# ratschlab/secedo

Hardware: AMD Instinct MI355X
Metric: cell-pair x locus updates/sec (similarity matrix) (higher is better)
Workload: dtype int64; 1 GPU; C3: 8000 cells x 100000 loci; entries=24345058, kept_entries=24223307, reads=23997029, block_cells=128, tiles=2016, normalization=ADD_MIN, max_fragment_length=1000, num_threads=8, parallelism=single GPU, backend=none, world_size=1, rccl_world_size=1

## Files before the change

### secedo_amd/csrc/simmat_kernels.hip

```cpp
#include "simmat_kernels.hpp"

#include <hip/hip_runtime.h>

#include <algorithm>
#include <type_traits>

namespace secedo {

uint32_t counts_split(uint32_t n_tiles);

namespace {

constexpr uint32_t META_PREV_OVF = 1u << 19;
constexpr uint32_t META_NEXT_OVF = 1u << 20;
constexpr uint32_t C_CELL = 127u;
constexpr uint32_t C_BASE_SHIFT = 7;
constexpr uint32_t C_TAIL = 1u << 9;
constexpr uint32_t C_MULTI = 1u << 10;
constexpr uint32_t C_WIDE = 1u << 11;
constexpr int LUT_DIM = 129;
constexpr int SLUT_DIM = 10;
constexpr long long NO_PAIR = (long long)0x8000000000000000ull;

__device__ __forceinline__ double log_add(double a, double b) {
    const double hi = fmax(a, b), lo = fmin(a, b);
    return hi + log1p(exp(lo - hi));
}

#ifdef SECEDO_STAMPS
__device__ __forceinline__ unsigned long long stamp() {
    unsigned long long t;
    asm volatile("s_memtime %0\n\ts_waitcnt lgkmcnt(0)" : "=s"(t)::"memory");
    return t;
}
__device__ __forceinline__ unsigned long long stamp_real() {
    unsigned long long t;
    asm volatile("s_memrealtime %0\n\ts_waitcnt lgkmcnt(0)" : "=s"(t)::"memory");
    return t;
}
#define STAMP(var) __builtin_amdgcn_sched_barrier(0); const unsigned long long var = stamp(); __builtin_amdgcn_sched_barrier(0)
#else
#define STAMP(var)
#endif

__device__ __forceinline__ uint32_t wave_inclusive_scan(uint32_t v) {
    v += __builtin_amdgcn_update_dpp(0u, v, 0x111, 0xF, 0xF, true);
    v += __builtin_amdgcn_update_dpp(0u, v, 0x112, 0xF, 0xF, true);
    v += __builtin_amdgcn_update_dpp(0u, v, 0x114, 0xF, 0xF, true);
    v += __builtin_amdgcn_update_dpp(0u, v, 0x118, 0xF, 0xF, true);
    v += __builtin_amdgcn_update_dpp(0u, v, 0x142, 0xA, 0xF, true);
    v += __builtin_amdgcn_update_dpp(0u, v, 0x143, 0xC, 0xF, true);
    return v;
}

constexpr uint32_t REF_TABLE_MAX = 128;
__device__ __noinline__ long long llr_fixed_device(const SlowPathArgs *sp, uint32_t xs, uint32_t xd, uint32_t cell_a,
                                                   uint32_t cell_b) {
    if (sp->beyond_list) {
        const uint32_t k = atomicAdd(sp->beyond_count, 1u);
        if (k < sp->beyond_cap) sp->beyond_list[k] = make_uint4(cell_a, cell_b, xs, xd);
        return 0ll;
    }
    const LlrModelDev m = sp->model;
    const int scale_log2 = sp->scale_log2;
    const double s = xs, d = xd;
    const double diff = log_add(s * m.ln_u1 + d * m.ln_v1, s * m.ln_u2 + d * m.ln_v2);
    const double same = log_add(s * m.ln_w1 + d * m.ln_z1, s * m.ln_w2 + d * m.ln_z2);
    return llrint(ldexp(diff - same, scale_log2));
}

__device__ __noinline__ long long slow_pair(const SlowPathArgs *sp, uint32_t r1, uint32_t r2,
                                            uint32_t locus, uint32_t cell_a, uint32_t cell_b) {
    const SlowPathArgs a = *sp;
    uint32_t i1 = a.read_off[r1], e1 = a.read_off[r1 + 1];
    uint32_t i2 = a.read_off[r2], e2 = a.read_off[r2 + 1];
    uint32_t xs = 0, xd = 0, first = 0xFFFFFFFFu;
    while (i1 < e1 && i2 < e2) {
        const uint32_t l1 = a.read_locus[i1], l2 = a.read_locus[i2];
        if (l1 == l2) {
            if (first == 0xFFFFFFFFu) first = l1;
            if (a.read_base[i1] == a.read_base[i2]) ++xs; else ++xd;
            ++i1; ++i2;
        } else if (l1 < l2) {
            ++i1;
        } else {
            ++i2;
        }
    }
    if (first != locus) return NO_PAIR;
    return xs + xd <= REF_TABLE_MAX ? a.lut[xs * LUT_DIM + xd] : llr_fixed_device(sp, xs, xd, cell_a, cell_b);
}

__device__ __noinline__ long long pair_value_full(const SlowPathArgs *sp, uint32_t g1, uint32_t g2) {
    const uint4 *entry = sp->entry;
    const uint4 A1 = entry[g1], A2 = entry[g2];
    if (A1.y & A2.y & 0xFFFFu) return NO_PAIR;
    const bool same = (((A1.x ^ A2.x) >> 16) & 3u) == 0u;
    if ((A1.x & A2.x & (META_PREV_OVF | META_NEXT_OVF)) == 0u) {
        const uint32_t shared = (A1.y & A2.y) >> 16;
        const uint32_t x = A1.z ^ A2.z;
        const uint32_t diff = ((x & 0xFFFFu) | (x >> 16)) & shared;
        const uint32_t nd = __popc(diff);
        const uint32_t xd = nd + (same ? 0u : 1u);
        const uint32_t xs = __popc(shared) - nd + (same ? 1u : 0u);
        return sp->lut[xs * LUT_DIM + xd];
    }
    const uint32_t *entry_read = sp->entry_read;
    return slow_pair(sp, entry_read[g1], entry_read[g2], A1.w, A1.x & 0xFFFFu, A2.x & 0xFFFFu);
}


struct TileChunk {
    uint32_t t;
    bool diag;
    uint32_t lane;
    const uint32_t *offI, *offJ;
    uint32_t r_begin, r_end;
    uint32_t row_begin, row_end;
};
template <int THREADS>
__device__ __forceinline__ TileChunk tile_chunk(const AccumulateArgs &a) {
    const uint32_t t_local = a.wg_tile[blockIdx.x];
    const uint32_t t = a.tile_ids ? a.tile_ids[t_local] : a.tile_begin + t_local;
    const uint32_t chunk = blockIdx.x - a.tile_wg_begin[t_local];
    const uint32_t n_chunks_t = a.tile_wg_begin[t_local + 1] - a.tile_wg_begin[t_local];
    const uint32_t I = a.tile_row[t], J = a.tile_col[t];
    const bool diag = (I == J);
    const uint32_t tid = threadIdx.x, lane = tid & 63u;
    const uint32_t *offI = a.blk_off + (size_t)I * a.stride;
    const uint32_t *offJ = a.blk_off + (size_t)J * a.stride;
    uint32_t r_begin = 0, r_end = a.num_ranges;
    uint32_t row_begin = 0u, row_end = 0xFFFFFFFFu;
    if (n_chunks_t > 1u) {
        const uint32_t L = a.stride - 1u;
        const uint32_t e0 = offI[0];
        const unsigned long long n_row = offI[L] - e0;
        row_begin = e0 + (uint32_t)(n_row * chunk / n_chunks_t);
        row_end = e0 + (uint32_t)(n_row * (chunk + 1u) / n_chunks_t);
        uint32_t before = 0, upto = 0;
        for (uint32_t base = 0; base < a.num_ranges; base += THREADS) {
            const uint32_t k = base + tid;
            bool ends_before = false, begins_inside = false;
            if (k < a.num_ranges) {
                ends_before = offI[a.range_off[k + 1u]] <= row_begin;
                begins_inside = offI[a.range_off[k]] < row_end;
            }
            before += (uint32_t)__syncthreads_count(ends_before);
            upto += (uint32_t)__syncthreads_count(begins_inside);
        }
        r_begin = __builtin_amdgcn_readfirstlane(before);
        r_end = __builtin_amdgcn_readfirstlane(upto);
        row_begin = __builtin_amdgcn_readfirstlane(row_begin);
        row_end = __builtin_amdgcn_readfirstlane(row_end);
    }
    return TileChunk{t, diag, lane, offI, offJ, r_begin, r_end, row_begin, row_end};
}

struct RangeCursor {
// ... 284 lines not shown
                            const bool ok = (!TAIL || pp[u] < total) && (both & C_TAIL) == 0u
                                    && ((x & cell_test) != 0u || !diag);
                            upd += ok ? 1u : 0u;
                            const uint32_t cell = (rr[u].x >> 16) + (ww[u] & C_CELL);
                            if (MCAP > 0) {
                                const bool joint = ok && (both & C_MULTI) != 0u;
                                const unsigned long long bal = __ballot(joint);
                                if (bal) {
                                    if (joint) {
                                        const uint32_t slot = n_list + __builtin_amdgcn_mbcnt_hi(
                                                (uint32_t)(bal >> 32), __builtin_amdgcn_mbcnt_lo((uint32_t)bal, 0u));
                                        mlist[slot] = make_uint2(ib + cur * 64u + oo[u], jb + rr[u].y + pp[u]);
                                        mcell[slot] = (uint16_t)cell;
                                    }
                                    n_list += (uint32_t)__popcll(bal);
                                }
                            } else {
                                multi_seen |= ok ? both : 0u;
                            }
                            if ((a.debug & 1u) == 0u && ok && (both & C_MULTI) == 0u) {
                                const bool differ = (x & (3u << C_BASE_SHIFT)) != 0u;
                                atomicAdd(&tile64[cell], (unsigned long long)(differ ? d01 : d10));
                            }
                        }
                    };
                    using two = std::integral_constant<int, 2>;
                    using one = std::integral_constant<int, 1>;
                    if (!(a.debug & 2u)) {
                        uint32_t base = 0;
                        for (; base + 128u <= total; base += 128u) trip(base, two{}, std::false_type{});
                        if (base < total) {
                            if (total - base <= 64u) trip(base, one{}, std::true_type{});
                            else trip(base, two{}, std::true_type{});
                        }
                    }
                    STAMP(t3);
#ifdef SECEDO_STAMPS
                    st_trip += t3 - t2;
                    st_t3 = t3;
#endif
                    const bool any_multi = MCAP == 0 && (multi_seen & C_MULTI) != 0u;
                    if (MCAP == 0 && __ballot(any_multi)) {
                        for (uint32_t p = lane; p < total; p += 64u) {
                            const uint32_t o = owner[p];
                            const uint2 ro = wrec[o];
                            const uint32_t jc = ro.y + p;
                            const uint32_t w = sJ[jc];
                            const uint32_t x = ro.x ^ w, both = ro.x & w;
                            const bool ok = (both & C_TAIL) == 0u && ((x & cell_test) != 0u || !diag);
                            if (ok && (both & C_MULTI) != 0u) {
                                const long long v = pair_value_full(a.slow, ib + cur * 64u + o, jb + jc);
                                const uint32_t cell = (ro.x >> 16) + (w & C_CELL);
                                if (v == NO_PAIR) ++skipped;
                                else atomicAdd(&tile64[cell], (unsigned long long)v);
                            }
                        }
                    }
                    __builtin_amdgcn_wave_barrier();
#ifdef SECEDO_STAMPS
                    { STAMP(t4); st_post += t4 - st_t3; }
#endif
                } else {
                    wrec[lane] = make_uint2(rec & 0xFFFFu, j0 - pex);
                    for (uint32_t win = 0; win < total; win += (uint32_t)HCAP) {
                        const uint32_t wlen = min((uint32_t)HCAP, total - win);
                        const uint32_t f0 = max(pex, win), f1 = min(pin, win + (uint32_t)HCAP);
                        for (uint32_t p = f0; p < f1; ++p) owner[p - win] = (unsigned char)lane;
                        __builtin_amdgcn_fence(__ATOMIC_RELEASE, "wavefront");
                        __builtin_amdgcn_wave_barrier();
                        for (uint32_t q = lane; q < wlen; q += 64u) {
                            const uint32_t o = owner[q];
                            const uint2 ro = wrec[o];
                            const uint32_t jc = ro.y + win + q;
                            pair(ro.x, sJ[jc], ib + cur * 64u + o, jb + jc);
                        }
                        __builtin_amdgcn_wave_barrier();
                    }
                }
                cur = nxt;
                rec = rec_n;
            }
        } else {
            pair_range_from_hbm<B, THREADS, false>(a, tc, la, ib, ie, dst, d10, d01, upd, skipped);
        }
#ifdef SECEDO_STAMPS
        { STAMP(te); st_loop += te - tb3; }
#endif
        const uint32_t upd_all = upd + (lane == 0u ? upd_w : 0u);
        n_updates += upd_all;
        n_pairs += (unsigned long long)upd_all - skipped;
    }
    STAMP(t_le);
    if (MCAP > 0 && n_list) flush_list();
    STAMP(t_fl);
    __syncthreads();
    STAMP(t_eb);

    {
        uint4 *out = reinterpret_cast<uint4 *>(reinterpret_cast<unsigned long long *>(a.slab) + (size_t)blockIdx.x * B * B);
        const uint4 *src = reinterpret_cast<const uint4 *>(tile64);
        for (uint32_t i = tid; i < B * B / 2; i += THREADS) out[i] = src[i];
    }

    STAMP(t_sl);
#ifdef SECEDO_STAMPS
    if (threadIdx.x == 0u && blockIdx.x < 2048u) {
        unsigned long long *w = a.counters + 16 + 2048 + (size_t)blockIdx.x * 8;
        w[0] = ((unsigned long long)__builtin_amdgcn_s_getreg((31 << 11) | 20) << 32)
                | (unsigned)__builtin_amdgcn_s_getreg((31 << 11) | 4);
        w[1] = t_le - t_pro;
        w[2] = t_fl - t_le;
        w[3] = t_eb - t_fl;
        w[4] = t_sl - t_eb;
        w[5] = st_real_begin;
        w[6] = stamp_real();
        w[7] = st_loop;
        a.counters[16 + blockIdx.x] = ((t_sl - st_begin) & 0xFFFFFFFFull) | ((unsigned long long)r_begin << 32)
                | ((unsigned long long)r_end << 44);
    }
#endif
    add_work_counters<WAVES>(a.counters, reinterpret_cast<unsigned long long *>(sJ), n_updates, n_pairs - skipped_list);
#ifdef SECEDO_STAMPS
    if (tid == 0u) {
        atomicAdd(&a.counters[2], st_setup);
        atomicAdd(&a.counters[3], st_fill);
        atomicAdd(&a.counters[4], st_trip);
        atomicAdd(&a.counters[5], st_batches);
        atomicAdd(&a.counters[6], st_trips);
        atomicAdd(&a.counters[7], stamp() - st_begin);
        atomicAdd(&a.counters[8], 1ull);
        atomicAdd(&a.counters[9], st_bar1);
        atomicAdd(&a.counters[10], st_stage);
        atomicAdd(&a.counters[11], st_pref);
        atomicAdd(&a.counters[12], st_post);
        atomicAdd(&a.counters[13], st_loop);
        atomicMax(&a.counters[14], stamp() - st_begin);
    }
#endif
}


constexpr int COUNTS_RING = 256;
constexpr uint32_t IT_J_SHIFT = 9, IT_C_SHIFT = 24, IT_J_MASK = 0x3FFFu, IT_WIDE = 32;
constexpr uint32_t IT_REC_MASK = 0x1FFu;

template <int B, int THREADS, int NCNT>
__device__ __forceinline__ void correct_epilogue(const AccumulateArgs &a, unsigned char *lds, uint32_t t_local,
                                                 const uint32_t (&cnt)[NCNT]);
template <bool WORDS>
__device__ __forceinline__ uint32_t counts_off_at(const uint16_t *sOff, uint32_t l) {
    if constexpr (WORDS) return (reinterpret_cast<const uint32_t *>(sOff)[l] >> IT_J_SHIFT) & IT_J_MASK;
    else return sOff[l];
}
template <int B, int THREADS, int CAPJ, int CAPL, int GROUP, bool WORDS>
__global__ __launch_bounds__(THREADS) void accumulate_counts(const AccumulateArgs a) {
    static_assert(CAPJ <= 16384, "14 bits of column index in an item");
    static_assert(GROUP >= 2 && GROUP <= 4, "group size");
    constexpr uint32_t ROW_WORDS = B + 1;
    constexpr size_t TILE_BYTES = ((size_t)B * ROW_WORDS * 4 + 15) / 16 * 16;
    constexpr int WAVES = THREADS / 64;
    constexpr int JPT = (CAPJ + THREADS - 1) / THREADS;
    constexpr int OPT = (CAPL + 1 + THREADS - 1) / THREADS;
    constexpr int RING = COUNTS_RING;

    extern __shared__ __attribute__((aligned(16))) unsigned char lds_raw[];
    uint32_t *tile32 = reinterpret_cast<uint32_t *>(lds_raw);
    uint32_t *sJ = reinterpret_cast<uint32_t *>(lds_raw + TILE_BYTES);
    uint16_t *sOff = reinterpret_cast<uint16_t *>(sJ + CAPJ);
    uint32_t *ring = reinterpret_cast<uint32_t *>(sOff + (CAPL + 2) * (WORDS ? 2 : 1)) + (threadIdx.x >> 6) * RING;

    const uint32_t t_local = a.wg_tile[blockIdx.x];
    const uint32_t t = a.tile_ids ? a.tile_ids[t_local] : a.tile_begin + t_local;
    const uint32_t chunk = blockIdx.x - a.tile_wg_begin[t_local];
    const uint32_t n_chunks_t = a.tile_wg_begin[t_local + 1] - a.tile_wg_begin[t_local];
    const uint32_t I = a.tile_row[t], J = a.tile_col[t];
    const bool diag = (I == J);
    const uint32_t tid = threadIdx.x, lane = tid & 63u;
    const uint32_t *offI = a.blk_off + (size_t)I * a.stride;
    const uint32_t *offJ = a.blk_off + (size_t)J * a.stride;
    uint32_t r_begin = 0, r_end = a.num_ranges;
    uint32_t row_begin = 0u, row_end = 0xFFFFFFFFu;
    if (n_chunks_t > 1u) {
        const uint32_t L = a.stride - 1u;
        const uint32_t e0 = offI[0];
        const unsigned long long n_row = offI[L] - e0;
        row_begin = e0 + (uint32_t)(n_row * chunk / n_chunks_t);
        row_end = e0 + (uint32_t)(n_row * (chunk + 1u) / n_chunks_t);
        uint32_t before = 0, upto = 0;
        for (uint32_t base = 0; base < a.num_ranges; base += THREADS) {
            const uint32_t k = base + tid;
            bool ends_before = false, begins_inside = false;
            if (k < a.num_ranges) {
                ends_before = offI[a.range_off[k + 1u]] <= row_begin;
                begins_inside = offI[a.range_off[k]] < row_end;
            }
            before += (uint32_t)__syncthreads_count(ends_before);
            upto += (uint32_t)__syncthreads_count(begins_inside);
        }
        r_begin = __builtin_amdgcn_readfirstlane(before);
        r_end = __builtin_amdgcn_readfirstlane(upto);
        row_begin = __builtin_amdgcn_readfirstlane(row_begin);
        row_end = __builtin_amdgcn_readfirstlane(row_end);
    }
    const TileChunk tc{t, diag, lane, offI, offJ, r_begin, r_end, row_begin, row_end};
    for (uint32_t i = tid; i < B * ROW_WORDS; i += THREADS) tile32[i] = 0u;

    unsigned long long n_updates = 0;
    uint32_t upd_w = 0;
    uint32_t ring_head = 0, ring_tail = 0;

    uint32_t pJ[JPT], pI[JPT], pO[OPT];
    uint32_t pO1[WORDS ? OPT : 1];
    RangeCursor nx;
    bool n_staged = false;
    auto prefetch = [&](uint32_t r) {
        nx.advance(a, tc, r);
        n_staged = (nx.je - nx.jb) <= (uint32_t)CAPJ && (nx.ie - nx.ib) <= (uint32_t)CAPJ
                && (nx.lb - nx.la) <= (uint32_t)CAPL;
        if (n_staged) {
            const __amdgpu_buffer_rsrc_t rj = __builtin_amdgcn_make_buffer_rsrc(
                    const_cast<uint32_t *>(a.entry32 + nx.jb), 0, (int)((nx.je - nx.jb) * 4u), 0x00020000);
            const __amdgpu_buffer_rsrc_t ro = __builtin_amdgcn_make_buffer_rsrc(
                    const_cast<uint32_t *>(offJ + nx.la), 0, (int)((nx.lb - nx.la + 1u) * 4u), 0x00020000);
#pragma unroll
            for (int k = 0; k < JPT; ++k)
                pJ[k] = (uint32_t)__builtin_amdgcn_raw_buffer_load_b32(rj, (int)(tid * 4u), k * THREADS * 4, 0);
#pragma unroll
            for (int k = 0; k < OPT; ++k)
                pO[k] = (uint32_t)__builtin_amdgcn_raw_buffer_load_b32(ro, (int)(tid * 4u), k * THREADS * 4, 0);
            if (WORDS) {
#pragma unroll
                for (int k = 0; k < OPT; ++k)
                    pO1[k] = (uint32_t)__builtin_amdgcn_raw_buffer_load_b32(ro, (int)(tid * 4u + 4u), k * THREADS * 4, 0);
            }
        }
    };
    auto prefetch_rows = [&]() {
        if (n_staged) {
            const __amdgpu_buffer_rsrc_t ri = __builtin_amdgcn_make_buffer_rsrc(
                    const_cast<uint32_t *>(a.entry32 + nx.ib), 0, (int)((nx.ie - nx.ib) * 4u), 0x00020000);
#pragma unroll
            for (int k = 0; k < JPT; ++k)
                pI[k] = (uint32_t)__builtin_amdgcn_raw_buffer_load_b32(ri, (int)(tid * 4u), k * THREADS * 4, 0);
        }
    };

    if (r_begin < r_end) {
        nx.prime(a, tc);
        prefetch(r_begin);
        prefetch_rows();
    }
#ifdef SECEDO_STAMPS
    unsigned long long st_barA = 0, st_stage = 0, st_items = 0, st_prim = 0, st_drain = 0, st_nprim = 0, st_ndrain = 0;
    const unsigned long long st_begin = stamp();
#endif
    {
        const bool DIAG = diag;
        const uint32_t lds_base = (uint32_t)reinterpret_cast<uintptr_t>(lds_raw);
        auto pair_slot = [&](uint32_t rec9, uint32_t row_byte, uint32_t w, unsigned long long in) {
            if (DIAG) in &= __ballot((w & 0xFFFFu) != ((rec9 & C_CELL) << 2));
            upd_w += (uint32_t)__popcll(in);
            const uint32_t addr = row_byte + (w & 0xFFFFu);
            if (__builtin_amdgcn_inverse_ballot_w64(in))
                atomicAdd(reinterpret_cast<uint32_t *>(lds_raw + addr),
                          (w >> 16) != (rec9 >> C_BASE_SHIFT) ? 0x10000u : 1u);
        };
        auto pair_slot_asm = [&](uint32_t rbase, uint32_t row_addr, uint32_t w, unsigned long long in) {
            upd_w += (uint32_t)__popcll(in);
            uint32_t addr, val;
            unsigned long long saved;
            asm volatile("s_and_saveexec_b64 %[saved], %[in]\n\t"
                         "v_cmp_eq_u32_sdwa vcc, %[w], %[rb] src0_sel:WORD_1 src1_sel:DWORD\n\t"
                         "v_add_u32_sdwa %[addr], %[row], %[w] dst_sel:DWORD dst_unused:UNUSED_PAD src0_sel:DWORD "
                         "src1_sel:WORD_0\n\t"
                         "s_nop 0\n\t"
                         "v_cndmask_b32_e64 %[val], %[k], 1, vcc\n\t"
                         "ds_add_u32 %[addr], %[val]\n\t"
                         "s_mov_b64 exec, %[saved]"
                         : [saved] "=&s"(saved), [addr] "=&v"(addr), [val] "=&v"(val)
                         : [in] "s"(in), [w] "v"(w), [rb] "v"(rbase), [row] "v"(row_addr), [k] "v"(0x10000u)
                         : "vcc", "memory");
        };

        auto group_load = [&](uint32_t item, uint32_t (&w)[GROUP]) {
            const uint32_t *p = sJ + ((item >> IT_J_SHIFT) & IT_J_MASK);
#pragma unroll
            for (int u = 0; u < GROUP; ++u) w[u] = p[u];
        };
        auto group_pair = [&](uint32_t item, const uint32_t (&w)[GROUP]) {
            const uint32_t c = item >> IT_C_SHIFT;
            const uint32_t rec9 = item & IT_REC_MASK;
            const uint32_t row_byte = (item & C_CELL) * (ROW_WORDS * 4u);
            unsigned long long in[GROUP];
#pragma unroll
            for (int u = 0; u < GROUP; ++u) in[u] = __ballot(c > (uint32_t)u);
            const unsigned long long more = __ballot(c > (uint32_t)GROUP);
            if (!DIAG && (GROUP == 4 || GROUP == 2)) {
                const uint32_t rbase = rec9 >> C_BASE_SHIFT, row_addr = lds_base + row_byte;
#pragma unroll
                for (int u = 0; u < GROUP; ++u) upd_w += (uint32_t)__popcll(in[u]);
                uint32_t a0, a1, a2, a3, v0, v1, v2, v3;
                unsigned long long saved, q0, q1, q2, q3;
                if (GROUP == 4) {
                    asm volatile("v_cmp_eq_u32_sdwa %[q0], %[w0], %[rb] src0_sel:WORD_1 src1_sel:DWORD\n\t"
                                 "v_cmp_eq_u32_sdwa %[q1], %[w1], %[rb] src0_sel:WORD_1 src1_sel:DWORD\n\t"
                                 "v_cmp_eq_u32_sdwa %[q2], %[w2], %[rb] src0_sel:WORD_1 src1_sel:DWORD\n\t"
                                 "v_cmp_eq_u32_sdwa %[q3], %[w3], %[rb] src0_sel:WORD_1 src1_sel:DWORD\n\t"
                                 "v_add_u32_sdwa %[a0], %[row], %[w0] dst_sel:DWORD dst_unused:UNUSED_PAD src0_sel:DWORD src1_sel:WORD_0\n\t"
                                 "v_add_u32_sdwa %[a1], %[row], %[w1] dst_sel:DWORD dst_unused:UNUSED_PAD src0_sel:DWORD src1_sel:WORD_0\n\t"
                                 "v_add_u32_sdwa %[a2], %[row], %[w2] dst_sel:DWORD dst_unused:UNUSED_PAD src0_sel:DWORD src1_sel:WORD_0\n\t"
                                 "v_add_u32_sdwa %[a3], %[row], %[w3] dst_sel:DWORD dst_unused:UNUSED_PAD src0_sel:DWORD src1_sel:WORD_0\n\t"
                                 "v_cndmask_b32_e64 %[v0], %[k], 1, %[q0]\n\t"
                                 "v_cndmask_b32_e64 %[v1], %[k], 1, %[q1]\n\t"
                                 "v_cndmask_b32_e64 %[v2], %[k], 1, %[q2]\n\t"
                                 "v_cndmask_b32_e64 %[v3], %[k], 1, %[q3]\n\t"
                                 "s_mov_b64 %[saved], exec\n\t"
                                 "s_mov_b64 exec, %[in0]\n\t"
                                 "ds_add_u32 %[a0], %[v0]\n\t"
                                 "s_mov_b64 exec, %[in1]\n\t"
                                 "ds_add_u32 %[a1], %[v1]\n\t"
                                 "s_mov_b64 exec, %[in2]\n\t"
                                 "ds_add_u32 %[a2], %[v2]\n\t"
                                 "s_mov_b64 exec, %[in3]\n\t"
                                 "ds_add_u32 %[a3], %[v3]\n\t"
                                 "s_mov_b64 exec, %[saved]"
                                 : [a0] "=&v"(a0), [a1] "=&v"(a1), [a2] "=&v"(a2), [a3] "=&v"(a3), [v0] "=&v"(v0), [v1] "=&v"(v1),
                                   [v2] "=&v"(v2), [v3] "=&v"(v3), [saved] "=&s"(saved), [q0] "=&s"(q0), [q1] "=&s"(q1),
                                   [q2] "=&s"(q2), [q3] "=&s"(q3)
                                 : [w0] "v"(w[0]), [w1] "v"(w[1 % GROUP]), [w2] "v"(w[2 % GROUP]), [w3] "v"(w[3 % GROUP]),
                                   [rb] "v"(rbase), [row] "v"(row_addr), [k] "v"(0x10000u), [in0] "s"(in[0]),
                                   [in1] "s"(in[1 % GROUP]), [in2] "s"(in[2 % GROUP]), [in3] "s"(in[3 % GROUP])
                                 : "memory");
                } else {
                    asm volatile("v_cmp_eq_u32_sdwa %[q0], %[w0], %[rb] src0_sel:WORD_1 src1_sel:DWORD\n\t"
                                 "v_cmp_eq_u32_sdwa %[q1], %[w1], %[rb] src0_sel:WORD_1 src1_sel:DWORD\n\t"
                                 "v_add_u32_sdwa %[a0], %[row], %[w0] dst_sel:DWORD dst_unused:UNUSED_PAD src0_sel:DWORD src1_sel:WORD_0\n\t"
                                 "v_add_u32_sdwa %[a1], %[row], %[w1] dst_sel:DWORD dst_unused:UNUSED_PAD src0_sel:DWORD src1_sel:WORD_0\n\t"
                                 "s_mov_b64 %[saved], exec\n\t"
                                 "v_cndmask_b32_e64 %[v0], %[k], 1, %[q0]\n\t"
                                 "v_cndmask_b32_e64 %[v1], %[k], 1, %[q1]\n\t"
                                 "s_mov_b64 exec, %[in0]\n\t"
                                 "ds_add_u32 %[a0], %[v0]\n\t"
                                 "s_mov_b64 exec, %[in1]\n\t"
                                 "ds_add_u32 %[a1], %[v1]\n\t"
                                 "s_mov_b64 exec, %[saved]"
                                 : [a0] "=&v"(a0), [a1] "=&v"(a1), [v0] "=&v"(v0), [v1] "=&v"(v1), [saved] "=&s"(saved),
                                   [q0] "=&s"(q0), [q1] "=&s"(q1)
                                 : [w0] "v"(w[0]), [w1] "v"(w[1 % GROUP]), [rb] "v"(rbase), [row] "v"(row_addr), [k] "v"(0x10000u),
                                   [in0] "s"(in[0]), [in1] "s"(in[1 % GROUP])
                                 : "memory");
                    (void)a2; (void)a3; (void)v2; (void)v3; (void)q2; (void)q3;
                }
            } else if (!DIAG) {
                const uint32_t rbase = rec9 >> C_BASE_SHIFT, row_addr = lds_base + row_byte;
#pragma unroll
                for (int u = 0; u < GROUP; ++u) pair_slot_asm(rbase, row_addr, w[u], in[u]);
            } else {
#pragma unroll
                for (int u = 0; u < GROUP; ++u) pair_slot(rec9, row_byte, w[u], in[u]);
            }
            if (more) {
                if (__builtin_amdgcn_inverse_ballot_w64(more)) {
                    const uint32_t slot = ring_tail + __builtin_amdgcn_mbcnt_hi(
                            (uint32_t)(more >> 32), __builtin_amdgcn_mbcnt_lo((uint32_t)more, 0u));
                    ring[slot & (RING - 1)] = item + ((uint32_t)GROUP << IT_J_SHIFT) - ((uint32_t)GROUP << IT_C_SHIFT);
                }
                ring_tail += (uint32_t)__popcll(more);
            }
        };
        auto group4 = [&](uint32_t item) {
            uint32_t w[GROUP];
            group_load(item, w);
            group_pair(item, w);
        };
        auto drain_one = [&]() {
            __builtin_amdgcn_fence(__ATOMIC_RELEASE, "wavefront");
            __builtin_amdgcn_wave_barrier();
            const uint32_t n = min(64u, ring_tail - ring_head);
            uint32_t it = 0u;
            if (lane < n) it = ring[(ring_head + lane) & (RING - 1)];
            __builtin_amdgcn_wave_barrier();
            ring_head += n;
            group4(it);
        };

        for (uint32_t r = r_begin; r < r_end; ++r) {
            const uint32_t la = nx.la, ib = nx.ib, ie = nx.ie, jb = nx.jb, dsh = nx.dsh;
            const bool staged = n_staged;
            STAMP(s0);
            __syncthreads();
            STAMP(s1);
            if (staged) {
                static_assert(JPT * THREADS <= CAPJ && OPT * THREADS <= CAPL + 2, "unconditional staging stores");
#pragma unroll
                for (int k = 0; k < JPT; ++k)
                    sJ[tid + k * THREADS] = ((pJ[k] & C_CELL) << 2) | ((pJ[k] << (16 - C_BASE_SHIFT)) & 0x30000u);
                if (WORDS) {
#pragma unroll
                    for (int k = 0; k < OPT; ++k)
                        reinterpret_cast<uint32_t *>(sOff)[tid + k * THREADS] = (((pO[k] - jb) & IT_J_MASK) << IT_J_SHIFT)
                                                | (min(pO1[k] - pO[k], 255u) << IT_C_SHIFT);
                } else {
#pragma unroll
                    for (int k = 0; k < OPT; ++k) sOff[tid + k * THREADS] = (uint16_t)(pO[k] - jb);
                }
            }
            __syncthreads();
            STAMP(s2);

            const uint32_t nI = ie - ib;
            upd_w = 0;
            if (staged) {
                uint32_t item[JPT];
                uint32_t any_wide = 0;
                if (WORDS && !DIAG) {
                    uint32_t word[JPT];
#pragma unroll
                    for (int k = 0; k < JPT; ++k) word[k] = reinterpret_cast<const uint32_t *>(sOff)[pI[k] >> 16];
#pragma unroll
                    for (int k = 0; k < JPT; ++k) {
                        item[k] = tid + k * THREADS < nI ? (pI[k] & IT_REC_MASK) | word[k] : 0u;
                        any_wide |= item[k];
                    }
                    any_wide >>= IT_C_SHIFT;
                } else {
#pragma unroll
                    for (int k = 0; k < JPT; ++k) {
                        const uint32_t i = tid + k * THREADS;
                        const uint32_t rec = pI[k];
                        const uint32_t lrel = rec >> 16;
                        uint32_t j0 = counts_off_at<WORDS>(sOff, lrel);
                        const uint32_t j1 = counts_off_at<WORDS>(sOff, lrel + 1);
                        if (DIAG) j0 = i + dsh + 1u;
                        const uint32_t c = (i < nI && j1 > j0) ? j1 - j0 : 0u;
                        any_wide |= c;
                        item[k] = (rec & IT_REC_MASK) | ((j0 & IT_J_MASK) << IT_J_SHIFT) | (c << IT_C_SHIFT);
                    }
                }
                if (__ballot(any_wide >= IT_WIDE)) {
#pragma unroll
                    for (int k = 0; k < JPT; ++k) {
                        const uint32_t i = tid + k * THREADS;
                        const uint32_t rec = pI[k];
                        const uint32_t lrel = rec >> 16;
                        uint32_t j0 = counts_off_at<WORDS>(sOff, lrel);
                        const uint32_t j1 = counts_off_at<WORDS>(sOff, lrel + 1);
                        if (DIAG) j0 = i + dsh + 1u;
                        const uint32_t c = (i < nI && j1 > j0) ? j1 - j0 : 0u;
                        unsigned long long todo = __ballot(c >= IT_WIDE);
                        while (todo) {
                            const int src = __builtin_ctzll(todo);
                            todo &= todo - 1ull;
                            const uint32_t recw = __builtin_amdgcn_readlane(rec, src);
                            const uint32_t cw = __builtin_amdgcn_readlane(c, src);
                            const uint32_t j0w = __builtin_amdgcn_readlane(j0, src);
                            const uint32_t row_byte = (recw & C_CELL) * (ROW_WORDS * 4u);
                            for (uint32_t base = 0; base < cw; base += 64u) {
                                const uint32_t jj = j0w + base + lane;
                                const unsigned long long in = __ballot(base + lane < cw);
                                const uint32_t w = sJ[min(jj, (uint32_t)CAPJ - 1u)];
                                pair_slot(recw & IT_REC_MASK, row_byte, w, in);
                            }
                        }
                        if (c >= IT_WIDE) item[k] = 0u;
                    }
                }
                if (r + 1 < r_end) prefetch(r + 1);
                STAMP(s3);
                {
                    uint32_t wc[GROUP], wn[GROUP];
                    group_load(item[0], wc);
#pragma unroll
                    for (int k = 0; k < JPT; ++k) {
                        if (k + 1 < JPT) group_load(item[k + 1], wn);
                        while (ring_tail - ring_head > (uint32_t)(RING - 64)) drain_one();
                        group_pair(item[k], wc);
#pragma unroll
                        for (int u = 0; u < GROUP; ++u) wc[u] = wn[u];
                    }
                }
                if (r + 1 < r_end) prefetch_rows();
                STAMP(s4);
#ifdef SECEDO_STAMPS
                st_ndrain += (ring_tail - ring_head + 63u) / 64u;
                st_nprim += JPT;
#endif
                while (ring_tail != ring_head) drain_one();
                STAMP(s5);
#ifdef SECEDO_STAMPS
                st_barA += s1 - s0;
                st_stage += s2 - s1;
                st_items += s3 - s2;
                st_prim += s4 - s3;
                st_drain += s5 - s4;
#endif
            } else {
                if (r + 1 < r_end) {
                    prefetch(r + 1);
                    prefetch_rows();
                }
                uint32_t upd = 0;
                for (uint32_t e1 = ib + tid; e1 < ie; e1 += THREADS) {
                    const uint32_t r1 = a.entry32[e1];
                    const uint32_t l = la + (r1 >> 16);
                    const uint32_t j0 = DIAG ? e1 + 1 : offJ[l];
                    const uint32_t j1 = offJ[l + 1];
                    const uint32_t row = (r1 & C_CELL) * ROW_WORDS;
                    for (uint32_t e2 = j0; e2 < j1; ++e2) {
                        const uint32_t r2 = a.entry32[e2];
                        const uint32_t x = r1 ^ r2;
                        if (DIAG && (x & C_CELL) == 0u) continue;
                        ++upd;
                        atomicAdd(&tile32[row + (r2 & C_CELL)], (x & (3u << C_BASE_SHIFT)) ? 0x10000u : 1u);
                    }
                }
                n_updates += upd;
            }
            if (lane == 0u) n_updates += upd_w;
        }
    }
#ifdef SECEDO_STAMPS
    if (lane == 0u && (blockIdx.x & 15u) == 0u) {
        atomicAdd(&a.counters[2], st_barA);
        atomicAdd(&a.counters[3], st_stage);
        atomicAdd(&a.counters[4], st_items);
        atomicAdd(&a.counters[5], st_prim);
        atomicAdd(&a.counters[6], st_drain);
        atomicAdd(&a.counters[7], stamp() - st_begin);
        atomicAdd(&a.counters[8], 1ull);
        atomicAdd(&a.counters[9], st_nprim);
        atomicAdd(&a.counters[10], st_ndrain);
        atomicAdd(&a.counters[16 + (tid >> 6) * 4 + 0], st_barA);
        atomicAdd(&a.counters[16 + (tid >> 6) * 4 + 1], st_prim + st_drain);
        atomicAdd(&a.counters[16 + (tid >> 6) * 4 + 2], st_items);
        atomicAdd(&a.counters[16 + (tid >> 6) * 4 + 3], st_stage);
    }
#endif
    __syncthreads();

    constexpr int NCNT = (B * B) / THREADS;
    static_assert(NCNT * THREADS == B * B && NCNT <= 16, "the count tile in whole words per thread");
    uint32_t cnt[NCNT];
    if (a.fused) {
#pragma unroll
        for (int k = 0; k < NCNT; ++k) {
            const uint32_t i = tid + (uint32_t)k * THREADS;
            cnt[k] = tile32[(i / B) * ROW_WORDS + (i % B)];
        }
    } else {
        uint32_t *out = reinterpret_cast<uint32_t *>(a.slab) + (size_t)blockIdx.x * B * B;
        for (uint32_t i = tid; i < B * B; i += THREADS) out[i] = tile32[(i / B) * ROW_WORDS + (i % B)];
    }
    for (int off = 32; off > 0; off >>= 1) n_updates += __shfl_down(n_updates, off);
    unsigned long long *red = reinterpret_cast<unsigned long long *>(sJ);
    if (lane == 0u) red[tid >> 6] = n_updates;
    __syncthreads();
    if (tid == 0u) {
        unsigned long long u = 0;
        for (int w = 0; w < WAVES; ++w) u += red[w];
        if (u) {
            atomicAdd(&a.counters[0], u);
            atomicAdd(&a.counters[1], u);
        }
    }
    if (a.fused) {
        __syncthreads();
        correct_epilogue<B, THREADS, NCNT>(a, lds_raw, t_local, cnt);
    }
}

constexpr int MASKS_RING = 128;
constexpr uint32_t MASKS_ROW_Q(int B) { return (uint32_t)B + 1u; }
constexpr uint32_t MK_J_MASK = 0xFFFu, MK_ROW_SHIFT = 12, MK_ROW_MASK = 0x7Fu, MK_C_SHIFT = 24;
constexpr uint32_t MX_PREV = 0xFFu << 16, MX_TAIL = 1u << 24, MX_DEAD = 1u << 26, MX_BASE = 0xFu << 28;
constexpr int MLUT_STRIDE = 11;
constexpr int MLUT_WORDS = 10 * MLUT_STRIDE;

__device__ __forceinline__ uint32_t masks_planes(uint32_t m) {
    const uint32_t n4 = __builtin_amdgcn_perm(m, m, 0x01010101u);
    const uint32_t b0 = __builtin_amdgcn_perm(m, m, 0x02020202u) ^ 0x00FF00FFu;
    const uint32_t b1 = __builtin_amdgcn_perm(m, m, 0x03030303u) ^ 0x0000FFFFu;
    return n4 & b0 & b1;
}
__device__ __forceinline__ uint32_t masks_flags(uint32_t e, uint32_t m) {
    const uint32_t base = (e >> C_BASE_SHIFT) & 3u;
    return ((m & 0xFFu) << 16) | ((e & (C_TAIL | C_WIDE)) << 15) | (0x10000000u << base);
}
static_assert((C_TAIL << 15) == MX_TAIL && (C_WIDE << 15) == MX_DEAD, "flag positions");

template <int B, int THREADS, int CAPJ, int CAPL, int GROUP>
__global__ __launch_bounds__(THREADS) void accumulate_masks(const AccumulateArgs a) {
    static_assert(CAPJ <= 4096, "12 bits of column index in an item");
    static_assert(GROUP == 3, "pair_group3_asm pairs three slots");
    constexpr uint32_t ROW_Q = MASKS_ROW_Q(B);
    constexpr size_t TILE_BYTES = (size_t)B * ROW_Q * 8;
    constexpr int WAVES = THREADS / 64;
    constexpr int JPT = (CAPJ + THREADS - 1) / THREADS;
    constexpr int OPT = (CAPL + 1 + THREADS - 1) / THREADS;
    constexpr int RING = MASKS_RING;

    extern __shared__ __attribute__((aligned(16))) unsigned char lds_raw[];
    unsigned long long *tile64 = reinterpret_cast<unsigned long long *>(lds_raw);
    uint2 *sJ = reinterpret_cast<uint2 *>(lds_raw + TILE_BYTES);
    uint16_t *sOff = reinterpret_cast<uint16_t *>(sJ + CAPJ);
    long long *sLut = reinterpret_cast<long long *>(sOff + CAPL + 2);
    uint2 *ring = reinterpret_cast<uint2 *>(sLut + MLUT_WORDS) + (threadIdx.x >> 6) * RING;
    uint32_t *ring_y = reinterpret_cast<uint32_t *>(reinterpret_cast<uint2 *>(sLut + MLUT_WORDS) + WAVES * RING)
            + (threadIdx.x >> 6) * RING;

    const TileChunk tc = tile_chunk<THREADS>(a);
    const uint32_t t = tc.t, r_begin = tc.r_begin, r_end = tc.r_end;
    const bool DIAG = tc.diag;
    const uint32_t tid = threadIdx.x, lane = tc.lane;
    const uint32_t *offJ = tc.offJ;
    for (uint32_t i = tid; i < B * ROW_Q; i += THREADS) tile64[i] = 0ull;
    for (uint32_t i = tid; i < (uint32_t)MLUT_WORDS; i += THREADS) {
        const uint32_t xs = i / MLUT_STRIDE, n = i % MLUT_STRIDE;
        sLut[i] = (n <= 8u && xs <= n + 1u) ? a.lut[xs * LUT_DIM + (n + 1u - xs)] : 0ll;
    }

    unsigned long long *dst = reinterpret_cast<unsigned long long *>(a.acc) + (size_t)t * B * B;
    unsigned long long n_updates = 0, n_pairs = 0;
    uint32_t upd_lane = 0, add_lane = 0;
    uint32_t ring_head = 0, ring_tail = 0;

    uint32_t pJ[JPT], pMj[JPT], pI[JPT], pXi[JPT], pMi[JPT], pO[OPT];
    RangeCursor nx;
    bool n_staged = false;
    auto prefetch = [&](uint32_t r) {
        nx.advance(a, tc, r);
        n_staged = (nx.je - nx.jb) <= (uint32_t)CAPJ && (nx.ie - nx.ib) <= (uint32_t)CAPJ
                && (nx.lb - nx.la) <= (uint32_t)CAPL;
// ... 1089 lines not shown
```

Measured before the change: 799.1 billion updates/s.

## Prefetch column words two groups ahead with asm ds_read2 and explicit lgkmcnt waits

Replaces the compiler-generated LDS loads of each group's column words with inline-asm ds_read2_b32 reads. Those words are now loaded two items ahead in a three-slot rotation, and each group's atomic block waits with a computed partial s_waitcnt lgkmcnt, so LDS reads overlap the preceding ds_add atomics instead of stalling on full waits. It also adds a dedicated asm path for GROUP==3, which previously fell back to per-slot asm. The risk is that the hand-computed lgkmcnt values are fragile: any LDS op the compiler schedules in between, such as the ring drain, could make the counts wrong or force conservative waits.

```diff
diff --git a/secedo_amd/csrc/simmat_kernels.hip b/secedo_amd/csrc/simmat_kernels.hip
--- a/secedo_amd/csrc/simmat_kernels.hip
+++ b/secedo_amd/csrc/simmat_kernels.hip
@@ -4,6 +4,7 @@
 
 #include <algorithm>
 #include <type_traits>
+#include <utility>
 
 namespace secedo {
 
@@ -594,6 +595,10 @@
     if constexpr (WORDS) return (reinterpret_cast<const uint32_t *>(sOff)[l] >> IT_J_SHIFT) & IT_J_MASK;
     else return sOff[l];
 }
+template <int... K, class F>
+__device__ __forceinline__ void for_each_index(std::integer_sequence<int, K...>, F &&f) {
+    (f(std::integral_constant<int, K>{}), ...);
+}
 template <int B, int THREADS, int CAPJ, int CAPL, int GROUP, bool WORDS>
 __global__ __launch_bounds__(THREADS) void accumulate_counts(const AccumulateArgs a) {
     static_assert(CAPJ <= 16384, "14 bits of column index in an item");
@@ -698,7 +703,8 @@
 #endif
     {
         const bool DIAG = diag;
-        const uint32_t lds_base = (uint32_t)reinterpret_cast<uintptr_t>(lds_raw);
+        const uint32_t lds_base = (uint32_t)reinterpret_cast<uintptr_t>(
+                (__attribute__((address_space(3))) unsigned char *)lds_raw);
         auto pair_slot = [&](uint32_t rec9, uint32_t row_byte, uint32_t w, unsigned long long in) {
             if (DIAG) in &= __ballot((w & 0xFFFFu) != ((rec9 & C_CELL) << 2));
             upd_w += (uint32_t)__popcll(in);
@@ -707,29 +713,25 @@
                 atomicAdd(reinterpret_cast<uint32_t *>(lds_raw + addr),
                           (w >> 16) != (rec9 >> C_BASE_SHIFT) ? 0x10000u : 1u);
         };
-        auto pair_slot_asm = [&](uint32_t rbase, uint32_t row_addr, uint32_t w, unsigned long long in) {
-            upd_w += (uint32_t)__popcll(in);
-            uint32_t addr, val;
-            unsigned long long saved;
-            asm volatile("s_and_saveexec_b64 %[saved], %[in]\n\t"
-                         "v_cmp_eq_u32_sdwa vcc, %[w], %[rb] src0_sel:WORD_1 src1_sel:DWORD\n\t"
-                         "v_add_u32_sdwa %[addr], %[row], %[w] dst_sel:DWORD dst_unused:UNUSED_PAD src0_sel:DWORD "
-                         "src1_sel:WORD_0\n\t"
-                         "s_nop 0\n\t"
-                         "v_cndmask_b32_e64 %[val], %[k], 1, vcc\n\t"
-                         "ds_add_u32 %[addr], %[val]\n\t"
-                         "s_mov_b64 exec, %[saved]"
-                         : [saved] "=&s"(saved), [addr] "=&v"(addr), [val] "=&v"(val)
-                         : [in] "s"(in), [w] "v"(w), [rb] "v"(rbase), [row] "v"(row_addr), [k] "v"(0x10000u)
-                         : "vcc", "memory");
+        constexpr int NREADS = GROUP == 2 ? 1 : 2;
+        struct Words {
+            unsigned long long w01, w23;
+            uint32_t w2;
         };
 
-        auto group_load = [&](uint32_t item, uint32_t (&w)[GROUP]) {
-            const uint32_t *p = sJ + ((item >> IT_J_SHIFT) & IT_J_MASK);
-#pragma unroll
-            for (int u = 0; u < GROUP; ++u) w[u] = p[u];
+        auto group_load = [&](uint32_t item, Words &w) {
+            const uint32_t pa = lds_base + (uint32_t)TILE_BYTES + (((item >> IT_J_SHIFT) & IT_J_MASK) << 2);
+            if constexpr (GROUP == 4)
+                asm volatile("ds_read2_b32 %0, %2 offset1:1\n\tds_read2_b32 %1, %2 offset0:2 offset1:3"
+                             : "=&v"(w.w01), "=v"(w.w23) : "v"(pa) : "memory");
+            else if constexpr (GROUP == 3)
+                asm volatile("ds_read2_b32 %0, %2 offset1:1\n\tds_read_b32 %1, %2 offset:8"
+                             : "=&v"(w.w01), "=v"(w.w2) : "v"(pa) : "memory");
+            else
+                asm volatile("ds_read2_b32 %0, %1 offset1:1" : "=v"(w.w01) : "v"(pa) : "memory");
         };
-        auto group_pair = [&](uint32_t item, const uint32_t (&w)[GROUP]) {
+        auto group_pair = [&](uint32_t item, Words &wd, auto wn_c) {
+            constexpr int WN = decltype(wn_c)::value;
             const uint32_t c = item >> IT_C_SHIFT;
             const uint32_t rec9 = item & IT_REC_MASK;
             const uint32_t row_byte = (item & C_CELL) * (ROW_WORDS * 4u);
@@ -737,14 +739,17 @@
 #pragma unroll
             for (int u = 0; u < GROUP; ++u) in[u] = __ballot(c > (uint32_t)u);
             const unsigned long long more = __ballot(c > (uint32_t)GROUP);
-            if (!DIAG && (GROUP == 4 || GROUP == 2)) {
+            if (!DIAG) {
                 const uint32_t rbase = rec9 >> C_BASE_SHIFT, row_addr = lds_base + row_byte;
 #pragma unroll
                 for (int u = 0; u < GROUP; ++u) upd_w += (uint32_t)__popcll(in[u]);
+                const uint32_t w0 = (uint32_t)wd.w01, w1 = (uint32_t)(wd.w01 >> 32);
                 uint32_t a0, a1, a2, a3, v0, v1, v2, v3;
                 unsigned long long saved, q0, q1, q2, q3;
-                if (GROUP == 4) {
-                    asm volatile("v_cmp_eq_u32_sdwa %[q0], %[w0], %[rb] src0_sel:WORD_1 src1_sel:DWORD\n\t"
+                if constexpr (GROUP == 4) {
+                    const uint32_t w2 = (uint32_t)wd.w23, w3 = (uint32_t)(wd.w23 >> 32);
+                    asm volatile("s_waitcnt lgkmcnt(%[wn])\n\t"
+                                 "v_cmp_eq_u32_sdwa %[q0], %[w0], %[rb] src0_sel:WORD_1 src1_sel:DWORD\n\t"
                                  "v_cmp_eq_u32_sdwa %[q1], %[w1], %[rb] src0_sel:WORD_1 src1_sel:DWORD\n\t"
                                  "v_cmp_eq_u32_sdwa %[q2], %[w2], %[rb] src0_sel:WORD_1 src1_sel:DWORD\n\t"
                                  "v_cmp_eq_u32_sdwa %[q3], %[w3], %[rb] src0_sel:WORD_1 src1_sel:DWORD\n\t"
@@ -769,12 +774,40 @@
                                  : [a0] "=&v"(a0), [a1] "=&v"(a1), [a2] "=&v"(a2), [a3] "=&v"(a3), [v0] "=&v"(v0), [v1] "=&v"(v1),
                                    [v2] "=&v"(v2), [v3] "=&v"(v3), [saved] "=&s"(saved), [q0] "=&s"(q0), [q1] "=&s"(q1),
                                    [q2] "=&s"(q2), [q3] "=&s"(q3)
-                                 : [w0] "v"(w[0]), [w1] "v"(w[1 % GROUP]), [w2] "v"(w[2 % GROUP]), [w3] "v"(w[3 % GROUP]),
+                                 : [w0] "v"(w0), [w1] "v"(w1), [w2] "v"(w2), [w3] "v"(w3),
                                    [rb] "v"(rbase), [row] "v"(row_addr), [k] "v"(0x10000u), [in0] "s"(in[0]),
-                                   [in1] "s"(in[1 % GROUP]), [in2] "s"(in[2 % GROUP]), [in3] "s"(in[3 % GROUP])
+                                   [in1] "s"(in[1 % GROUP]), [in2] "s"(in[2 % GROUP]), [in3] "s"(in[3 % GROUP]), [wn] "n"(WN)
                                  : "memory");
+                } else if constexpr (GROUP == 3) {
+                    const uint32_t w2 = wd.w2;
+                    asm volatile("s_waitcnt lgkmcnt(%[wn])\n\t"
+                                 "v_cmp_eq_u32_sdwa %[q0], %[w0], %[rb] src0_sel:WORD_1 src1_sel:DWORD\n\t"
+                                 "v_cmp_eq_u32_sdwa %[q1], %[w1], %[rb] src0_sel:WORD_1 src1_sel:DWORD\n\t"
+                                 "v_cmp_eq_u32_sdwa %[q2], %[w2], %[rb] src0_sel:WORD_1 src1_sel:DWORD\n\t"
+                                 "v_add_u32_sdwa %[a0], %[row], %[w0] dst_sel:DWORD dst_unused:UNUSED_PAD src0_sel:DWORD src1_sel:WORD_0\n\t"
+                                 "v_add_u32_sdwa %[a1], %[row], %[w1] dst_sel:DWORD dst_unused:UNUSED_PAD src0_sel:DWORD src1_sel:WORD_0\n\t"
+                                 "v_add_u32_sdwa %[a2], %[row], %[w2] dst_sel:DWORD dst_unused:UNUSED_PAD src0_sel:DWORD src1_sel:WORD_0\n\t"
+                                 "s_mov_b64 %[saved], exec\n\t"
+                                 "v_cndmask_b32_e64 %[v0], %[k], 1, %[q0]\n\t"
+                                 "v_cndmask_b32_e64 %[v1], %[k], 1, %[q1]\n\t"
+                                 "v_cndmask_b32_e64 %[v2], %[k], 1, %[q2]\n\t"
+                                 "s_mov_b64 exec, %[in0]\n\t"
+                                 "ds_add_u32 %[a0], %[v0]\n\t"
+                                 "s_mov_b64 exec, %[in1]\n\t"
+                                 "ds_add_u32 %[a1], %[v1]\n\t"
+                                 "s_mov_b64 exec, %[in2]\n\t"
+                                 "ds_add_u32 %[a2], %[v2]\n\t"
+                                 "s_mov_b64 exec, %[saved]"
+                                 : [a0] "=&v"(a0), [a1] "=&v"(a1), [a2] "=&v"(a2), [v0] "=&v"(v0), [v1] "=&v"(v1), [v2] "=&v"(v2),
+                                   [saved] "=&s"(saved), [q0] "=&s"(q0), [q1] "=&s"(q1), [q2] "=&s"(q2)
+                                 : [w0] "v"(w0), [w1] "v"(w1), [w2] "v"(w2), [rb] "v"(rbase), [row] "v"(row_addr),
+                                   [k] "v"(0x10000u), [in0] "s"(in[0]), [in1] "s"(in[1 % GROUP]), [in2] "s"(in[2 % GROUP]),
+                                   [wn] "n"(WN)
+                                 : "memory");
+                    (void)a3; (void)v3; (void)q3;
                 } else {
-                    asm volatile("v_cmp_eq_u32_sdwa %[q0], %[w0], %[rb] src0_sel:WORD_1 src1_sel:DWORD\n\t"
+                    asm volatile("s_waitcnt lgkmcnt(%[wn])\n\t"
+                                 "v_cmp_eq_u32_sdwa %[q0], %[w0], %[rb] src0_sel:WORD_1 src1_sel:DWORD\n\t"
                                  "v_cmp_eq_u32_sdwa %[q1], %[w1], %[rb] src0_sel:WORD_1 src1_sel:DWORD\n\t"
                                  "v_add_u32_sdwa %[a0], %[row], %[w0] dst_sel:DWORD dst_unused:UNUSED_PAD src0_sel:DWORD src1_sel:WORD_0\n\t"
                                  "v_add_u32_sdwa %[a1], %[row], %[w1] dst_sel:DWORD dst_unused:UNUSED_PAD src0_sel:DWORD src1_sel:WORD_0\n\t"
@@ -788,18 +821,22 @@
                                  "s_mov_b64 exec, %[saved]"
                                  : [a0] "=&v"(a0), [a1] "=&v"(a1), [v0] "=&v"(v0), [v1] "=&v"(v1), [saved] "=&s"(saved),
                                    [q0] "=&s"(q0), [q1] "=&s"(q1)
-                                 : [w0] "v"(w[0]), [w1] "v"(w[1 % GROUP]), [rb] "v"(rbase), [row] "v"(row_addr), [k] "v"(0x10000u),
-                                   [in0] "s"(in[0]), [in1] "s"(in[1 % GROUP])
+                                 : [w0] "v"(w0), [w1] "v"(w1), [rb] "v"(rbase), [row] "v"(row_addr), [k] "v"(0x10000u),
+                                   [in0] "s"(in[0]), [in1] "s"(in[1 % GROUP]), [wn] "n"(WN)
                                  : "memory");
                     (void)a2; (void)a3; (void)v2; (void)v3; (void)q2; (void)q3;
                 }
-            } else if (!DIAG) {
-                const uint32_t rbase = rec9 >> C_BASE_SHIFT, row_addr = lds_base + row_byte;
-#pragma unroll
-                for (int u = 0; u < GROUP; ++u) pair_slot_asm(rbase, row_addr, w[u], in[u]);
             } else {
-#pragma unroll
-                for (int u = 0; u < GROUP; ++u) pair_slot(rec9, row_byte, w[u], in[u]);
+                if constexpr (GROUP == 4) asm volatile("s_waitcnt lgkmcnt(0)" : "+v"(wd.w01), "+v"(wd.w23)::"memory");
+                else if constexpr (GROUP == 3) asm volatile("s_waitcnt lgkmcnt(0)" : "+v"(wd.w01), "+v"(wd.w2)::"memory");
+                else asm volatile("s_waitcnt lgkmcnt(0)" : "+v"(wd.w01)::"memory");
+                pair_slot(rec9, row_byte, (uint32_t)wd.w01, in[0]);
+                pair_slot(rec9, row_byte, (uint32_t)(wd.w01 >> 32), in[1]);
+                if constexpr (GROUP == 3) pair_slot(rec9, row_byte, wd.w2, in[2 % GROUP]);
+                if constexpr (GROUP == 4) {
+                    pair_slot(rec9, row_byte, (uint32_t)wd.w23, in[2 % GROUP]);
+                    pair_slot(rec9, row_byte, (uint32_t)(wd.w23 >> 32), in[3 % GROUP]);
+                }
             }
             if (more) {
                 if (__builtin_amdgcn_inverse_ballot_w64(more)) {
@@ -811,9 +848,9 @@
             }
         };
         auto group4 = [&](uint32_t item) {
-            uint32_t w[GROUP];
+            Words w;
             group_load(item, w);
-            group_pair(item, w);
+            group_pair(item, w, std::integral_constant<int, 0>{});
         };
         auto drain_one = [&]() {
             __builtin_amdgcn_fence(__ATOMIC_RELEASE, "wavefront");
@@ -910,16 +947,17 @@
                 if (r + 1 < r_end) prefetch(r + 1);
                 STAMP(s3);
                 {
-                    uint32_t wc[GROUP], wn[GROUP];
-                    group_load(item[0], wc);
-#pragma unroll
-                    for (int k = 0; k < JPT; ++k) {
-                        if (k + 1 < JPT) group_load(item[k + 1], wn);
+                    Words ws[3];
+                    group_load(item[0], ws[0]);
+                    if (JPT > 1) group_load(item[1 % JPT], ws[1]);
+                    for_each_index(std::make_integer_sequence<int, JPT>{}, [&](auto kc) {
+                        constexpr int k = decltype(kc)::value;
+                        if constexpr (k + 2 < JPT) group_load(item[k + 2], ws[(k + 2) % 3]);
                         while (ring_tail - ring_head > (uint32_t)(RING - 64)) drain_one();
-                        group_pair(item[k], wc);
-#pragma unroll
-                        for (int u = 0; u < GROUP; ++u) wc[u] = wn[u];
-                    }
+                        constexpr int WN = (k >= 2 ? GROUP : 0) + (k >= 1 ? GROUP : 0) + (k + 1 < JPT ? NREADS : 0)
+                                         + (k + 2 < JPT ? NREADS : 0);
+                        group_pair(item[k], ws[k % 3], std::integral_constant<int, WN>{});
+                    });
                 }
                 if (r + 1 < r_end) prefetch_rows();
                 STAMP(s4);
```

New measurement: 810.4 billion updates/s (median of 6 runs). 1.4% higher.
